# oso95/Agentainer-lab

Measured on AMD Instinct MI355X. Metric: concurrent_agent_chat_req_per_s, higher is better.
Workload: dtype bf16; 1 GPU; model=llama3-8b, agents_per_gpu=64, agents=64, global_batch=64, prompt_len=256, gen_len=57, seq_len=313, parallelism=dp1

## Files before the change

### agentainer_amd/models/llama.py

```python

from __future__ import annotations

import math
from dataclasses import dataclass
from typing import Dict, List, Optional

import torch
import torch.nn.functional as F

from .. import ops


@dataclass
class LlamaConfig:
    name: str = "tiny-llama"
    vocab_size: int = 512
    hidden_size: int = 512
    n_layers: int = 2
    n_heads: int = 4
    n_kv_heads: int = 1
    head_dim: int = 128
    intermediate_size: int = 1024
    rope_theta: float = 500000.0
    max_position: int = 8192
# ... 2 lines not shown
    qkv_bias: bool = False

    @property
    def q_size(self):
        return self.n_heads * self.head_dim

    @property
    def kv_size(self):
        return self.n_kv_heads * self.head_dim

    def kv_bytes_per_token(self, dtype_bytes: int = 2) -> int:
        return 2 * self.n_layers * self.n_kv_heads * self.head_dim * dtype_bytes


@dataclass
class AttnMetadata:

    page_table: torch.Tensor
    seq_lens: torch.Tensor
    slot_mapping: torch.Tensor
    positions: torch.Tensor
    is_prefill: bool = False
    query_starts: Optional[torch.Tensor] = None
    query_lens: Optional[torch.Tensor] = None
    max_qlen: int = 0


class LlamaAttention(torch.nn.Module):
    def __init__(self, cfg: LlamaConfig, tp_rank: int = 0, tp_size: int = 1):
        super().__init__()
        assert cfg.n_heads % tp_size == 0, "n_heads must divide tp_size"
        assert cfg.n_kv_heads % tp_size == 0 or tp_size == 1, \
            "n_kv_heads must divide tp_size"
        self.cfg = cfg
        self.tp_size = tp_size
        self.n_heads = cfg.n_heads // tp_size
        self.n_kv = max(cfg.n_kv_heads // tp_size, 1)
        self.head_dim = cfg.head_dim
        self.scale = 1.0 / math.sqrt(cfg.head_dim)
        q_out = self.n_heads * cfg.head_dim
        kv_out = self.n_kv * cfg.head_dim
        self.qkv_proj = torch.nn.Parameter(
            torch.empty(q_out + 2 * kv_out, cfg.hidden_size, dtype=torch.bfloat16))
        self.o_proj = torch.nn.Parameter(
            torch.empty(cfg.hidden_size, q_out, dtype=torch.bfloat16))
        self.qkv_bias = (torch.nn.Parameter(
            torch.zeros(q_out + 2 * kv_out, dtype=torch.bfloat16))
            if cfg.qkv_bias else None)
        self.qkv_packed = None
        self.o_packed = None
        self.qkv_q = None
        self.o_q = None

    def forward(self, h, k_cache, v_cache, md: AttnMetadata, cos_sin, tp_group=None):
        T = h.size(0)
        if self.qkv_q is not None and T <= 64 and h.is_cuda:
            qkv = ops.linear_quant(h, self.qkv_q)
        else:
            qkv = ops.linear(h, self.qkv_proj, self.qkv_packed)
        if self.qkv_bias is not None:
            qkv = qkv + self.qkv_bias
        q_sz = self.n_heads * self.head_dim
        kv_sz = self.n_kv * self.head_dim
        q = qkv[:, :q_sz].view(T, self.n_heads, self.head_dim)
        k = qkv[:, q_sz:q_sz + kv_sz].view(T, self.n_kv, self.head_dim)
        v = qkv[:, q_sz + kv_sz:].view(T, self.n_kv, self.head_dim)
        ops.rope_append(q, k, v, k_cache, v_cache, cos_sin, md.positions,
                        md.slot_mapping)
        out = torch.empty(T, self.n_heads, self.head_dim, dtype=q.dtype,
                          device=q.device)
        if md.is_prefill:
            ops.paged_prefill_attention(out, q, k_cache, v_cache, md.page_table,
                                        md.seq_lens, md.query_starts,
                                        md.query_lens, self.scale,
                                        max_qlen=md.max_qlen)
        else:
            ops.paged_decode_attention(out, q, k_cache, v_cache, md.page_table,
                                       md.seq_lens, self.scale)
        if self.o_q is not None and T <= 64 and h.is_cuda:
            o = ops.linear_quant(out.view(T, q_sz), self.o_q)
        else:
            o = ops.linear(out.view(T, q_sz), self.o_proj, self.o_packed)
        if tp_group is not None:
            torch.distributed.all_reduce(o, group=tp_group)
        return o


class LlamaMLP(torch.nn.Module):
    def __init__(self, cfg: LlamaConfig, tp_size: int = 1):
        super().__init__()
        inter = cfg.intermediate_size // tp_size
        self.gate_up = torch.nn.Parameter(
            torch.empty(2 * inter, cfg.hidden_size, dtype=torch.bfloat16))
        self.down = torch.nn.Parameter(
            torch.empty(cfg.hidden_size, inter, dtype=torch.bfloat16))
        self.inter = inter
        self.gate_up_packed = None
        self.down_packed = None
        self.gate_up_q = None
        self.down_q = None

    def forward(self, h, tp_group=None):
        turbo = self.gate_up_q is not None and h.size(0) <= 64 and h.is_cuda
        if turbo:
            gu = ops.linear_quant(h, self.gate_up_q)
        else:
            gu = ops.linear(h, self.gate_up, self.gate_up_packed)
        gate, up = gu[:, :self.inter], gu[:, self.inter:]
        act = torch.empty(gu.size(0), self.inter, dtype=gu.dtype,
                          device=gu.device)
        ops.silu_mul(act, gate, up)
        if turbo:
            out = ops.linear_quant(act, self.down_q)
        else:
            out = ops.linear(act, self.down, self.down_packed)
        if tp_group is not None:
            torch.distributed.all_reduce(out, group=tp_group)
        return out


class LlamaLayer(torch.nn.Module):
    def __init__(self, cfg: LlamaConfig, tp_rank: int = 0, tp_size: int = 1):
        super().__init__()
        self.attn = LlamaAttention(cfg, tp_rank, tp_size)
        self.mlp = LlamaMLP(cfg, tp_size)
        self.input_ln = torch.nn.Parameter(torch.empty(cfg.hidden_size, dtype=torch.bfloat16))
        self.post_ln = torch.nn.Parameter(torch.empty(cfg.hidden_size, dtype=torch.bfloat16))
        self.eps = cfg.norm_eps

    def forward(self, hidden, residual, k_cache, v_cache, md, cos_sin, tp_group=None):
        normed = torch.empty_like(hidden)
        if residual is None:
            residual = hidden.clone()
            ops.rmsnorm(normed, hidden, self.input_ln, self.eps)
        else:
            ops.fused_add_rmsnorm(normed, hidden, residual, self.input_ln, self.eps)
        attn_out = self.attn(normed, k_cache, v_cache, md, cos_sin, tp_group)
        normed2 = torch.empty_like(hidden)
        ops.fused_add_rmsnorm(normed2, attn_out, residual, self.post_ln, self.eps)
        mlp_out = self.mlp(normed2, tp_group)
        return mlp_out, residual


class LlamaForCausalLM(torch.nn.Module):
    def __init__(self, cfg: LlamaConfig, device="cpu", tp_rank: int = 0,
                 tp_size: int = 1, seed: int = 0):
        super().__init__()
        self.cfg = cfg
        self.tp_rank = tp_rank
        self.tp_size = tp_size
        self.tp_group = None
        with torch.device(device):
            self.embed = torch.nn.Parameter(
                torch.empty(cfg.vocab_size, cfg.hidden_size, dtype=torch.bfloat16))
            self.layers = torch.nn.ModuleList(
                [LlamaLayer(cfg, tp_rank, tp_size) for _ in range(cfg.n_layers)])
            self.final_ln = torch.nn.Parameter(
                torch.empty(cfg.hidden_size, dtype=torch.bfloat16))
            if cfg.tie_embeddings:
                self.lm_head = self.embed
            else:
                self.lm_head = torch.nn.Parameter(
                    torch.empty(cfg.vocab_size, cfg.hidden_size, dtype=torch.bfloat16))
        self.register_buffer(
            "cos_sin",
            ops.make_cos_sin_table(cfg.max_position, cfg.head_dim, cfg.rope_theta,
                                   device=device),
            persistent=False)
        self.random_init(seed)

    @torch.no_grad()
    def random_init(self, seed: int = 0):
        dev = self.embed.device
        gen = torch.Generator(device=dev).manual_seed(seed)
        for name, p in self.named_parameters():
            if p.dim() >= 2:
                p.data.normal_(0.0, 0.02, generator=gen)
            else:
                p.fill_(1.0)

    @torch.no_grad()
    def forward(self, input_ids: torch.Tensor, md: AttnMetadata,
                kv_caches: List, last_rows: Optional[torch.Tensor] = None
                ) -> torch.Tensor:
        hidden = F.embedding(input_ids, self.embed)
        residual = None
        for i, layer in enumerate(self.layers):
            k_cache, v_cache = kv_caches[i]
            hidden, residual = layer(hidden, residual, k_cache, v_cache, md,
                                     self.cos_sin, self.tp_group)
        final = torch.empty_like(hidden)
        ops.fused_add_rmsnorm(final, hidden, residual, self.final_ln, self.cfg.norm_eps)
        if last_rows is not None:
            final = final[last_rows]
        return ops.linear(final, self.lm_head,
                          getattr(self, 'lm_head_packed', None))

    @torch.no_grad()
    def pack_decode_weights(self, dense_quant: str = ""):
        for layer in self.layers:
            if dense_quant == "mxfp4":
                for mod_, wname, qname in (
                        (layer.attn, "qkv_proj", "qkv_q"),
                        (layer.attn, "o_proj", "o_q"),
                        (layer.mlp, "gate_up", "gate_up_q"),
                        (layer.mlp, "down", "down_q")):
                    w = getattr(mod_, wname).data
                    p, sc = ops.quantize_weight_mxfp4(w)
                    setattr(mod_, qname, ("mxfp4", p, sc, w.size(0)))
            elif dense_quant == "fp8":
                for mod_, wname, qname in (
                        (layer.attn, "qkv_proj", "qkv_q"),
                        (layer.attn, "o_proj", "o_q"),
                        (layer.mlp, "gate_up", "gate_up_q"),
                        (layer.mlp, "down", "down_q")):
                    w = getattr(mod_, wname).data
                    p, sw = ops.quantize_weight_fp8(w)
                    setattr(mod_, qname, ("fp8", p, sw, w.size(0)))
            else:
                layer.attn.qkv_packed = ops.pack_weight(layer.attn.qkv_proj.data)
                layer.attn.o_packed = ops.pack_weight(layer.attn.o_proj.data)
                layer.mlp.gate_up_packed = ops.pack_weight(layer.mlp.gate_up.data)
                layer.mlp.down_packed = ops.pack_weight(layer.mlp.down.data)
        self.lm_head_packed = ops.pack_weight(
            self.lm_head.data if isinstance(self.lm_head, torch.nn.Parameter)
            else self.lm_head)

    @torch.no_grad()
    def load_safetensors(self, path: str):
        from safetensors.torch import load_file
        import glob, os

        files = sorted(glob.glob(os.path.join(path, "*.safetensors")))
        if not files:
            raise FileNotFoundError(f"no safetensors under {path}")
        sd = {}
        for f in files:
            sd.update(load_file(f))
        self._load_hf_state_dict(sd)

    @torch.no_grad()
    def _load_hf_state_dict(self, sd: Dict[str, torch.Tensor]):
        cfg = self.cfg
        r, s = self.tp_rank, self.tp_size
# ... 93 lines not shown
```

### agentainer_amd/models/mixtral.py

```python

from __future__ import annotations

from dataclasses import dataclass
from typing import Dict, List, Optional

import torch
import torch.nn.functional as F

from .. import ops
from .llama import AttnMetadata, LlamaAttention, LlamaConfig


@dataclass
class MixtralConfig(LlamaConfig):
    n_experts: int = 8
    top_k: int = 2


class MixtralMoE(torch.nn.Module):

    def __init__(self, cfg: MixtralConfig, ep_rank: int = 0, ep_size: int = 1):
        super().__init__()
        assert cfg.n_experts % ep_size == 0
        self.cfg = cfg
# ... 153 lines not shown
                             device=h.device)
            le = md[:, 1].long()
            for i in range(self.n_local):
                sel = (le == i).nonzero(as_tuple=True)[0]
                if sel.numel() == 0:
                    continue
                xi = xd[sel]
                gu = ops.linear(xi, self.gate_up[i], None)
                gate, up = gu[:, :self.inter], gu[:, self.inter:]
                act = torch.empty(xi.shape[0], self.inter, dtype=gu.dtype,
                                  device=gu.device)
                ops.silu_mul(act, gate, up)
                eo = ops.linear(act, self.down[i], None)
                yd[sel] = md[sel, 2].unsqueeze(1) * eo.float()
            results.append(yd.to(h.dtype).contiguous())
        returned = self._exchange(results, ep_group)
        out_shard = torch.zeros(ts, H, dtype=torch.float32, device=h.device)
        for d in range(world):
            md = send_meta[d]
            if md.shape[0]:
                out_shard.index_add_(0, md[:, 0].long(),
                                     returned[d].float())
        shards = [None] * world
        sizes = [base + (1 if r < rem else 0) for r in range(world)]
        out_shard = out_shard.to(h.dtype)
        if dist.get_backend(ep_group) == "nccl" and len(set(sizes)) == 1:
            full = torch.empty(T, H, dtype=h.dtype, device=h.device)
            dist.all_gather_into_tensor(full.view(world, -1).view(-1),
                                        out_shard.contiguous(), group=ep_group)
            return full
        dist.all_gather_object(shards, out_shard.cpu(), group=ep_group)
        return torch.cat([s.to(h.device) for s in shards], dim=0)


class MixtralLayer(torch.nn.Module):
    def __init__(self, cfg: MixtralConfig, tp_rank: int = 0, tp_size: int = 1):
        super().__init__()
        self.attn = LlamaAttention(cfg, tp_rank, tp_size)
        self.moe = MixtralMoE(cfg, ep_rank=tp_rank, ep_size=tp_size)
        self.input_ln = torch.nn.Parameter(
            torch.empty(cfg.hidden_size, dtype=torch.bfloat16))
        self.post_ln = torch.nn.Parameter(
            torch.empty(cfg.hidden_size, dtype=torch.bfloat16))
        self.eps = cfg.norm_eps

    def forward(self, hidden, residual, k_cache, v_cache, md, cos_sin,
                tp_group=None):
        normed = torch.empty_like(hidden)
        if residual is None:
            residual = hidden.clone()
            ops.rmsnorm(normed, hidden, self.input_ln, self.eps)
        else:
            ops.fused_add_rmsnorm(normed, hidden, residual, self.input_ln, self.eps)
        attn_out = self.attn(normed, k_cache, v_cache, md, cos_sin, tp_group)
        normed2 = torch.empty_like(hidden)
        ops.fused_add_rmsnorm(normed2, attn_out, residual, self.post_ln, self.eps)
        moe_out = self.moe(normed2, ep_group=tp_group)
        return moe_out, residual


class MixtralForCausalLM(torch.nn.Module):
    def __init__(self, cfg: MixtralConfig, device="cpu", tp_rank: int = 0,
                 tp_size: int = 1, seed: int = 0):
        super().__init__()
        self.cfg = cfg
        self.tp_rank = tp_rank
        self.tp_size = tp_size
        self.tp_group = None
        with torch.device(device):
            self.embed = torch.nn.Parameter(
                torch.empty(cfg.vocab_size, cfg.hidden_size, dtype=torch.bfloat16))
            self.layers = torch.nn.ModuleList(
                [MixtralLayer(cfg, tp_rank, tp_size) for _ in range(cfg.n_layers)])
            self.final_ln = torch.nn.Parameter(
                torch.empty(cfg.hidden_size, dtype=torch.bfloat16))
            self.lm_head = torch.nn.Parameter(
                torch.empty(cfg.vocab_size, cfg.hidden_size, dtype=torch.bfloat16))
        self.register_buffer(
            "cos_sin",
            ops.make_cos_sin_table(cfg.max_position, cfg.head_dim,
                                   cfg.rope_theta, device=device),
            persistent=False)
        self.random_init(seed)

    @torch.no_grad()
    def random_init(self, seed: int = 0):
        dev = self.embed.device
        gen = torch.Generator(device=dev).manual_seed(seed)
        for name, p in self.named_parameters():
            if p.dim() >= 2:
                p.data.normal_(0.0, 0.02, generator=gen)
            else:
                p.fill_(1.0)

    @torch.no_grad()
    def pack_decode_weights(self, expert_fp8: bool = False,
                            expert_fp4: bool = False):
        for layer in self.layers:
            layer.attn.qkv_packed = ops.pack_weight(layer.attn.qkv_proj.data)
            layer.attn.o_packed = ops.pack_weight(layer.attn.o_proj.data)
            for i in range(layer.moe.n_local):
                if expert_fp4:
                    layer.moe.gate_up_fp4[i] = ops.quantize_weight_mxfp4(
                        layer.moe.gate_up[i].data)
                    layer.moe.down_fp4[i] = ops.quantize_weight_mxfp4(
                        layer.moe.down[i].data)
                elif expert_fp8:
# ... 59 lines not shown
```

### agentainer_amd/ops/__init__.py

```python

from __future__ import annotations

import os
from typing import Optional

import torch

from . import reference

_hip = None
_hip_err: Optional[str] = None


def _load_hip():
    global _hip, _hip_err
    if _hip is not None or _hip_err is not None:
        return _hip
    so = os.path.join(os.path.dirname(__file__), "_hip_ops.so")
    if not os.path.exists(so):
        _hip_err = f"HIP extension not built ({so} missing); run python -m agentainer_amd.ops.build"
        return None
    try:
        import importlib.util

        spec = importlib.util.spec_from_file_location("agentainer_amd.ops._hip_ops", so)
        mod = importlib.util.module_from_spec(spec)
        spec.loader.exec_module(mod)
        _hip = mod
    except Exception as exc:
        _hip_err = f"HIP extension failed to load: {exc}"
    return _hip


def hip_available() -> bool:
    return _load_hip() is not None


def _dispatch(name: str, *tensors: torch.Tensor):
    if tensors[0].is_cuda:
        mod = _load_hip()
        if mod is None:
            raise RuntimeError(
                f"op {name!r} on GPU requires the gfx950 HIP extension: {_hip_err}")
        return mod
    return None


def rmsnorm(out, x, w, eps: float = 1e-5):
    mod = _dispatch("rmsnorm", x)
    if mod:
        mod.rmsnorm(out, x, w, float(eps))
    else:
        reference.rmsnorm(out, x, w, eps)
    return out


def fused_add_rmsnorm(out, x, residual, w, eps: float = 1e-5):
    mod = _dispatch("fused_add_rmsnorm", x)
    if mod:
        mod.fused_add_rmsnorm(out, x, residual, w, float(eps))
    else:
        reference.fused_add_rmsnorm(out, x, residual, w, eps)
    return out


def silu_mul(out, gate, up):
    mod = _dispatch("silu_mul", gate)
    if mod:
        mod.silu_mul(out, gate, up)
    else:
        reference.silu_mul(out, gate, up)
    return out


make_cos_sin_table = reference.make_cos_sin_table


def rope_inplace(q, k, cos_sin, positions):
    mod = _dispatch("rope_inplace", q)
    if mod:
        mod.rope_inplace(q, k, cos_sin, positions)
    else:
        reference.rope_inplace(q, k, cos_sin, positions)


def rope_append(q, k, v, k_cache, v_cache, cos_sin, positions, slot_mapping):
    mod = _dispatch("rope_append", q)
    if mod:
        mod.rope_append(q, k, v, k_cache, v_cache, cos_sin, positions,
                        slot_mapping)
    else:
        reference.rope_inplace(q, k, cos_sin, positions)
        reference.kv_append(k_cache, v_cache, k, v, slot_mapping)


def kv_append(k_cache, v_cache, k, v, slot_mapping):
    mod = _dispatch("kv_append", k)
    if mod:
        mod.kv_append(k_cache, v_cache, k, v, slot_mapping)
    else:
        reference.kv_append(k_cache, v_cache, k, v, slot_mapping)


def paged_decode_attention(out, q, k_cache, v_cache, page_table, seq_lens,
                           scale: float):
    mod = _dispatch("paged_decode_attention", q)
    if mod:
        mod.paged_decode_attention(out, q, k_cache, v_cache, page_table,
                                   seq_lens, float(scale))
    else:
        reference.paged_decode_attention(out, q, k_cache, v_cache, page_table,
                                         seq_lens, scale)
    return out


def paged_prefill_attention(out, q, k_cache, v_cache, page_table, seq_lens,
                            query_starts, query_lens, scale: float,
                            max_qlen: int = 0):
    mod = _dispatch("paged_prefill_attention", q)
    if mod:
        mod.paged_prefill_attention(out, q, k_cache, v_cache, page_table,
                                    seq_lens, query_starts, query_lens,
                                    float(scale), int(max_qlen))
    else:
        reference.paged_prefill_attention(out, q, k_cache, v_cache, page_table,
                                          seq_lens, query_starts, query_lens,
                                          scale)
    return out


def greedy_sample(out, logits):
    mod = _dispatch("greedy_sample", logits)
    if mod:
        mod.greedy_sample(out, logits)
    else:
        reference.greedy_sample(out, logits)
    return out


def topp_sample(out, logits, temps, top_ps, seeds):
    mod = _dispatch("topp_sample", logits)
    if mod:
        mod.topp_sample(out, logits, temps, top_ps, seeds)
    else:
        reference.topp_sample(out, logits, temps, top_ps, seeds)
    return out


_ws_cache = {}
_EMPTY_WS = {}
SKINNY_DISABLED = os.environ.get("AGENTAINER_DISABLE_SKINNY", "0") == "1"
SKINNY_FORCED = os.environ.get("AGENTAINER_FORCE_SKINNY", "0") == "1"
_SKINNY_SHAPES = {
    (4096, 4096): (4, 128),
    (4096, 14336): (8, 128),
}
SKINNY_NT = os.environ.get("AGENTAINER_SKINNY_NT", "0") == "1"
SKINNY_KC = int(os.environ.get("AGENTAINER_SKINNY_KC", "0"))
for _spec in os.environ.get("AGENTAINER_SKINNY_SHAPES", "").split(","):
    if _spec.strip():
        _n, _k, _s, _c = (int(v) for v in _spec.split(":"))
        _SKINNY_SHAPES[(_n, _k)] = (_s, _c)


def _skinny_split(ntiles: int, K: int) -> int:
    split = 1
    while split < 16 and ntiles * split < 256 and K % (256 * split * 2) == 0:
        split *= 2
    return split


def pack_weight(w: torch.Tensor) -> torch.Tensor:
    N, K = w.shape
    assert N % 16 == 0 and K % 32 == 0
    p = w.view(N // 16, 16, K // 32, 4, 8).permute(0, 2, 3, 1, 4).contiguous()
    return p.view(-1)


def _skinny_ws(device, N: int, split: int) -> torch.Tensor:
    if split > 1:
        key = (device, N, split)
        ws = _ws_cache.get(key)
        if ws is None or ws.numel() < split * 64 * N:
            ws = torch.empty(split * 64 * N, dtype=torch.float32, device=device)
            _ws_cache[key] = ws
        return ws
    ws = _EMPTY_WS.get(device)
    if ws is None:
        ws = torch.empty(1, dtype=torch.float32, device=device)
        _EMPTY_WS[device] = ws
    return ws


def linear(x: torch.Tensor, w: torch.Tensor,
           w_packed: Optional[torch.Tensor] = None) -> torch.Tensor:
    M, K = x.shape
    N = w.size(0)
    tuned = _SKINNY_SHAPES.get((N, K))
    if (x.is_cuda and M <= 64 and N % 64 == 0 and K % 256 == 0
            and (tuned is not None or SKINNY_FORCED) and not SKINNY_DISABLED):
        mod = _dispatch("skinny_gemm", x)
        split, kc = tuned if tuned else (_skinny_split(N // 64, K), 128)
        if SKINNY_KC:
            kc = SKINNY_KC
        if K % (kc * split):
            split = _skinny_split(N // 64, K)
        out = torch.empty(M, N, dtype=x.dtype, device=x.device)
        ws = _skinny_ws(x.device, N, split)
        if w_packed is not None:
            mod.skinny_gemm_packed(out, x.contiguous(), w_packed, N, K, ws,
                                   split, SKINNY_NT, kc)
        else:
            mod.skinny_gemm(out, x.contiguous(), w, ws, split)
        return out
    return torch.nn.functional.linear(x, w)


def quantize_weight_fp8(w: torch.Tensor):
    N, K = w.shape
    sw = w.float().abs().amax(dim=1).clamp(min=1e-8) / 448.0
    scaled = (w.float() / sw[:, None]).clamp(-448.0, 448.0)
    try:
        w8 = scaled.to(torch.float8_e4m3fn).view(torch.uint8)
    except (RuntimeError, TypeError):
        w8 = scaled.cpu().to(torch.float8_e4m3fn).view(torch.uint8).to(w.device)
    packed = (w8.view(N // 16, 16, K // 32, 4, 8)
              .permute(0, 2, 3, 1, 4).contiguous().view(-1))
    return packed, sw.float().contiguous()


def linear_fp8(x: torch.Tensor, w_packed: torch.Tensor, sw: torch.Tensor,
               N: int) -> torch.Tensor:
    M, K = x.shape
    mod = _dispatch("skinny_gemm_fp8", x)
    assert mod is not None, "linear_fp8 is GPU-only"
    xc = x.contiguous()
    x8 = torch.empty(M, K, dtype=torch.uint8, device=x.device)
    sx = torch.empty(M, dtype=torch.float32, device=x.device)
    mod.quant_fp8_rows(x8, sx, xc)
    split = _skinny_split(N // 64, K)
    ws = _skinny_ws(x.device, N, split)
    out = torch.empty(M, N, dtype=x.dtype, device=x.device)
    mod.skinny_gemm_fp8(out, x8, sx, w_packed, sw, N, K, ws, split)
    return out


_FP4_GRID = torch.tensor([0.0, 0.5, 1.0, 1.5, 2.0, 3.0, 4.0, 6.0])
MXFP4_COMBO = int(os.environ.get("AGENTAINER_MXFP4_COMBO", "0"))


def quantize_weight_mxfp4(w: torch.Tensor):
    N, K = w.shape
    assert N % 16 == 0 and K % 128 == 0, "MXFP4: N%16==0, K%128==0"
    wf = w.float().view(N, K // 32, 32)
    amax = wf.abs().amax(dim=-1).clamp(min=1e-8)
    e = torch.ceil(torch.log2(amax / 6.0)).clamp(-127, 127)
    scale = torch.pow(2.0, e)
    q = wf / scale.unsqueeze(-1)
    mids = torch.tensor([0.25, 0.75, 1.25, 1.75, 2.5, 3.5, 5.0],
                        device=wf.device)
    idx = torch.bucketize(q.abs().contiguous(), mids)
    codes = (idx + torch.where(q < 0, 8, 0)).to(torch.uint8).view(N, K)
    by = (codes[:, 0::2] | (codes[:, 1::2] << 4))
    byv = by.view(N // 16, 16, K // 128, 4, 16)
    packed = byv.permute(0, 2, 3, 1, 4).contiguous().view(-1)
    e8 = (e + 127).clamp(0, 254).to(torch.uint8).view(N, K // 32)
    scv = e8.view(N // 16, 16, K // 128, 4).permute(0, 2, 3, 1).contiguous()
# ... 56 lines not shown
```

### agentainer_amd/ops/csrc/bindings.cpp

```cpp
#include <torch/extension.h>

void rmsnorm(torch::Tensor out, torch::Tensor x, torch::Tensor w, double eps);
void fused_add_rmsnorm(torch::Tensor out, torch::Tensor x,
                       torch::Tensor residual, torch::Tensor w, double eps);
void silu_mul(torch::Tensor out, torch::Tensor gate, torch::Tensor up);
void rope_inplace(torch::Tensor q, torch::Tensor k, torch::Tensor cos_sin,
                  torch::Tensor positions);
void rope_append(torch::Tensor q, torch::Tensor k, torch::Tensor v,
                 torch::Tensor k_cache, torch::Tensor v_cache,
                 torch::Tensor cos_sin, torch::Tensor positions,
                 torch::Tensor slot_mapping);
void kv_append(torch::Tensor k_cache, torch::Tensor v_cache, torch::Tensor k,
               torch::Tensor v, torch::Tensor slot_mapping);
void paged_decode_attention(torch::Tensor out, torch::Tensor q,
                            torch::Tensor k_cache, torch::Tensor v_cache,
                            torch::Tensor page_table, torch::Tensor seq_lens,
                            double scale);
void paged_prefill_attention(torch::Tensor out, torch::Tensor q,
                             torch::Tensor k_cache, torch::Tensor v_cache,
                             torch::Tensor page_table, torch::Tensor seq_lens,
                             torch::Tensor query_starts, torch::Tensor query_lens,
                             double scale, long max_qlen);
void greedy_sample(torch::Tensor out, torch::Tensor logits);
void topp_sample(torch::Tensor out, torch::Tensor logits, torch::Tensor temps,
                 torch::Tensor top_ps, torch::Tensor seeds);
void gather_kv_pages(torch::Tensor dst, torch::Tensor k_cache,
                     torch::Tensor v_cache, torch::Tensor page_ids);
void skinny_gemm(torch::Tensor out, torch::Tensor x, torch::Tensor w,
                 torch::Tensor ws, long split);
void skinny_gemm_packed(torch::Tensor out, torch::Tensor x,
                        torch::Tensor w_packed, long N, long K,
                        torch::Tensor ws, long split, bool nt, long kc);
void quant_fp8_rows(torch::Tensor x8, torch::Tensor sx, torch::Tensor x);
void quant_fp4_rows(torch::Tensor x4, torch::Tensor sx, torch::Tensor x);
void skinny_gemm_mxfp4(torch::Tensor out, torch::Tensor x8, torch::Tensor sx,
                       torch::Tensor w_packed, torch::Tensor w_scales, long N,
                       long K, torch::Tensor ws, long split, long combo);
void skinny_gemm_fp8(torch::Tensor out, torch::Tensor x8, torch::Tensor sx,
                     torch::Tensor w_packed, torch::Tensor sw, long N, long K,
                     torch::Tensor ws, long split);
void mfma_probe(torch::Tensor c, torch::Tensor a, torch::Tensor b);
void scatter_kv_pages(torch::Tensor k_cache, torch::Tensor v_cache,
                      torch::Tensor src, torch::Tensor page_ids);

PYBIND11_MODULE(TORCH_EXTENSION_NAME, m) {
  m.doc() = "agentainer_amd CDNA4 (gfx950) kernels";
  m.def("rmsnorm", &rmsnorm, "RMSNorm (bf16)");
  m.def("fused_add_rmsnorm", &fused_add_rmsnorm, "residual += x; rmsnorm");
  m.def("silu_mul", &silu_mul, "silu(gate) * up");
  m.def("rope_inplace", &rope_inplace, "apply rotary embedding to q,k in place");
  m.def("rope_append", &rope_append, "fused RoPE + paged KV append");
  m.def("kv_append", &kv_append, "scatter new k/v into the paged KV cache");
  m.def("paged_decode_attention", &paged_decode_attention,
        "single-token GQA attention over the paged KV cache");
  m.def("paged_prefill_attention", &paged_prefill_attention,
        "varlen causal MFMA attention over the paged KV cache");
  m.def("greedy_sample", &greedy_sample, "argmax over vocab per row");
  m.def("topp_sample", &topp_sample, "temperature + top-p sampling per row");
  m.def("gather_kv_pages", &gather_kv_pages, "pages -> host-shaped buffer");
  m.def("skinny_gemm", &skinny_gemm, "out[M,N] = x[M,K] @ W[N,K]^T, M<=64");
  m.def("skinny_gemm_packed", &skinny_gemm_packed, "packed-weight skinny GEMM");
  m.def("skinny_gemm_mxfp4", &skinny_gemm_mxfp4, "MXFP4 block-scaled expert GEMM");
  m.def("quant_fp4_rows", &quant_fp4_rows, "per-row e2m1 activation quant");
  m.def("quant_fp8_rows", &quant_fp8_rows, "per-row bf16 -> e4m3 quant");
  m.def("skinny_gemm_fp8", &skinny_gemm_fp8, "fp8 MFMA skinny GEMM");
  m.def("mfma_probe", &mfma_probe, "single 16x16x32 bf16 MFMA on prepacked fragments");
  m.def("scatter_kv_pages", &scatter_kv_pages, "buffer -> pages");
}
```

### agentainer_amd/ops/csrc/rmsnorm.hip

```cpp

#include <torch/extension.h>
#include <ATen/hip/HIPContext.h>
#include "common.h"

namespace {

template <bool FUSED_ADD, int VPT>
__global__ __launch_bounds__(512) void rmsnorm_kernel(
    short* __restrict__ out, const short* __restrict__ x,
    short* __restrict__ residual, const short* __restrict__ w, float eps,
    int H) {
  const int row = blockIdx.x;
  const int tid = threadIdx.x;
  const long base = (long)row * H;
  __shared__ float red[8];

  bf16x8 v[VPT];
  float ss = 0.f;
#pragma unroll
  for (int r = 0; r < VPT; ++r) {
    const int i = (tid + r * 512) * 8;
    if (i < H) {
      v[r] = *reinterpret_cast<const bf16x8*>(x + base + i);
      if (FUSED_ADD) {
        bf16x8 rv = *reinterpret_cast<const bf16x8*>(residual + base + i);
#pragma unroll
        for (int j = 0; j < 8; ++j)
          v[r][j] = f2bits(bits2f(v[r][j]) + bits2f(rv[j]));
        *reinterpret_cast<bf16x8*>(residual + base + i) = v[r];
      }
#pragma unroll
      for (int j = 0; j < 8; ++j) {
        const float f = bits2f(v[r][j]);
        ss = fmaf(f, f, ss);
      }
    } else {
      v[r] = bf16x8{};
    }
  }
  ss = wave_sum(ss);
  if ((tid & (WAVE - 1)) == 0) red[tid / WAVE] = ss;
  __syncthreads();
  ss = 0.f;
#pragma unroll
  for (int wv = 0; wv < 8; ++wv) ss += red[wv];
  const float rms = rsqrtf(ss / (float)H + eps);

#pragma unroll
  for (int r = 0; r < VPT; ++r) {
    const int i = (tid + r * 512) * 8;
    if (i < H) {
      bf16x8 wv = *reinterpret_cast<const bf16x8*>(w + i);
      bf16x8 ov;
#pragma unroll
      for (int j = 0; j < 8; ++j)
        ov[j] = f2bits(bits2f(v[r][j]) * rms * bits2f(wv[j]));
      *reinterpret_cast<bf16x8*>(out + base + i) = ov;
    }
  }
}

}

void rmsnorm(torch::Tensor out, torch::Tensor x, torch::Tensor w, double eps) {
  TORCH_CHECK(x.is_contiguous() && out.is_contiguous() && w.is_contiguous());
  TORCH_CHECK(x.scalar_type() == at::kBFloat16, "rmsnorm: bf16 only");
  const int H = x.size(-1);
  TORCH_CHECK(H % 8 == 0, "hidden size must be a multiple of 8");
  const int T = x.numel() / H;
  auto stream = at::hip::getCurrentHIPStream();
#define RN_LAUNCH(VPT)                                                         \
  hipLaunchKernelGGL((rmsnorm_kernel<false, VPT>), dim3(T), dim3(512), 0,      \
                     stream, (short*)out.data_ptr(),                           \
                     (const short*)x.data_ptr(), nullptr,                      \
                     (const short*)w.data_ptr(), (float)eps, H)
  if (H <= 4096) RN_LAUNCH(1);
  else if (H <= 8192) RN_LAUNCH(2);
  else if (H <= 16384) RN_LAUNCH(4);
  else TORCH_CHECK(false, "rmsnorm: hidden > 16384 unsupported");
#undef RN_LAUNCH
}

void fused_add_rmsnorm(torch::Tensor out, torch::Tensor x,
                       torch::Tensor residual, torch::Tensor w, double eps) {
  TORCH_CHECK(x.is_contiguous() && out.is_contiguous() && w.is_contiguous() &&
              residual.is_contiguous());
  TORCH_CHECK(x.scalar_type() == at::kBFloat16, "fused_add_rmsnorm: bf16 only");
  const int H = x.size(-1);
  TORCH_CHECK(H % 8 == 0, "hidden size must be a multiple of 8");
  const int T = x.numel() / H;
  auto stream = at::hip::getCurrentHIPStream();
#define RNF_LAUNCH(VPT)                                                        \
  hipLaunchKernelGGL((rmsnorm_kernel<true, VPT>), dim3(T), dim3(512), 0,       \
                     stream, (short*)out.data_ptr(),                           \
                     (const short*)x.data_ptr(), (short*)residual.data_ptr(),  \
                     (const short*)w.data_ptr(), (float)eps, H)
  if (H <= 4096) RNF_LAUNCH(1);
  else if (H <= 8192) RNF_LAUNCH(2);
  else if (H <= 16384) RNF_LAUNCH(4);
  else TORCH_CHECK(false, "rmsnorm: hidden > 16384 unsupported");
#undef RNF_LAUNCH
}
```

### agentainer_amd/ops/csrc/skinny_gemm.hip

```cpp

#include <torch/extension.h>
#include <ATen/hip/HIPContext.h>
#include "common.h"

namespace {

typedef __bf16 bf16v8 __attribute__((ext_vector_type(8)));

template <bool SPLIT, bool FULL>
__global__ __launch_bounds__(256) void skinny_gemm_kernel(
    void* __restrict__ out,
    const short* __restrict__ x,
    const short* __restrict__ w,
    int M, int N, int K, int k_per_split) {
  const int n0 = blockIdx.x * 64 + (threadIdx.x / WAVE) * 16;
  const int split = blockIdx.y;
  const int lane = threadIdx.x % WAVE;
  const int l16 = lane % 16;
  const int lg = lane / 16;
  const int k0 = split * k_per_split;
  const int k1 = min(k0 + k_per_split, K);

  f32x4 acc[4];
#pragma unroll
// ... 50 lines not shown
        acc[ms] = __builtin_amdgcn_mfma_f32_16x16x32_bf16(a[ms], bw[i],
                                                          acc[ms], 0, 0, 0);
    }
    if (has_next) stage_write(buf ^ 1);
    __syncthreads();
    buf ^= 1;
  }

#pragma unroll
  for (int ms = 0; ms < 4; ++ms) {
#pragma unroll
    for (int r = 0; r < 4; ++r) {
      const int row = ms * 16 + lg * 4 + r;
      if (row >= M) continue;
      const int col = blockIdx.x * 64 + (threadIdx.x / WAVE) * 16 + l16;
      if (SPLIT) {
        float* o = reinterpret_cast<float*>(out);
        o[((long)split * M + row) * N + col] = acc[ms][r];
      } else {
        short* o = reinterpret_cast<short*>(out);
        o[(long)row * N + col] = f2bits(acc[ms][r]);
      }
    }
  }
}

__global__ __launch_bounds__(256) void splitk_combine_kernel(
    short* __restrict__ out, const float* __restrict__ ws, long mn, int S) {
  const long i4 = ((long)blockIdx.x * blockDim.x + threadIdx.x) * 4;
  if (i4 >= mn) return;
  if (i4 + 4 <= mn) {
    f32x4 acc = *reinterpret_cast<const f32x4*>(ws + i4);
    for (int s = 1; s < S; ++s) {
      const f32x4 v = *reinterpret_cast<const f32x4*>(ws + (long)s * mn + i4);
#pragma unroll
      for (int j = 0; j < 4; ++j) acc[j] += v[j];
    }
    bf16x4 o;
#pragma unroll
    for (int j = 0; j < 4; ++j) o[j] = f2bits(acc[j]);
    *reinterpret_cast<bf16x4*>(out + i4) = o;
  } else {
    for (long i = i4; i < mn; ++i) {
      float acc = 0.f;
      for (int s = 0; s < S; ++s) acc += ws[(long)s * mn + i];
      out[i] = f2bits(acc);
    }
  }
}

}

void skinny_gemm(torch::Tensor out, torch::Tensor x, torch::Tensor w,
                 torch::Tensor ws, long split) {
  TORCH_CHECK(x.is_contiguous() && w.is_contiguous() && out.is_contiguous());
  TORCH_CHECK(x.scalar_type() == at::kBFloat16 && w.scalar_type() == at::kBFloat16);
  const int M = x.size(0), K = x.size(1), N = w.size(0);
  TORCH_CHECK(w.size(1) == K);
  TORCH_CHECK(M <= 64, "skinny_gemm: M <= 64");
  TORCH_CHECK(N % 64 == 0, "skinny_gemm: N % 64 == 0");
  TORCH_CHECK(K % 256 == 0, "skinny_gemm: K % 256 == 0");
  auto stream = at::hip::getCurrentHIPStream();
  const int ntiles = N / 64;
  TORCH_CHECK(split >= 1 && (K % (256 * split)) == 0,
              "invalid split for K (k slices must be 256-aligned)");
  const int kps = K / (int)split;
  const bool full = (M == 64);
#define SG_LAUNCH(SPLIT_, FULL_, OUTP)                                         \
  hipLaunchKernelGGL((skinny_gemm_kernel<SPLIT_, FULL_>),                      \
                     dim3(ntiles, SPLIT_ ? (int)split : 1), dim3(256), 0,      \
                     stream, OUTP, (const short*)x.data_ptr(),                 \
                     (const short*)w.data_ptr(), M, N, K, kps)
  if (split == 1) {
    if (full) SG_LAUNCH(false, true, out.data_ptr());
    else SG_LAUNCH(false, false, out.data_ptr());
  } else {
    TORCH_CHECK(ws.numel() >= (long)split * M * N,
                "skinny_gemm split-K workspace too small");
    TORCH_CHECK(ws.scalar_type() == at::kFloat);
    if (full) SG_LAUNCH(true, true, ws.data_ptr());
    else SG_LAUNCH(true, false, ws.data_ptr());
    const long mn = (long)M * N;
    hipLaunchKernelGGL(splitk_combine_kernel,
                       dim3((mn + 1023) / 1024), dim3(256), 0, stream,
                       (short*)out.data_ptr(), ws.data_ptr<float>(), mn, split);
  }
#undef SG_LAUNCH
}


namespace {

template <bool SPLIT, bool FULL, bool NT, int KC>
__global__ __launch_bounds__(256) void skinny_gemm_packed_kernel(
    void* __restrict__ out, const short* __restrict__ x,
    const short* __restrict__ wp_packed, int M, int N, int K,
    int k_per_split) {
  const int n_tile = blockIdx.x * 4 + threadIdx.x / WAVE;
  const int split = blockIdx.y;
  const int lane = threadIdx.x % WAVE;
  const int l16 = lane % 16;
  const int lg = lane / 16;
  const int k0 = split * k_per_split;
  const int k1 = min(k0 + k_per_split, K);

  f32x4 acc[4];
#pragma unroll
  for (int ms = 0; ms < 4; ++ms) acc[ms] = f32x4{0.f, 0.f, 0.f, 0.f};

  const short* wp = wp_packed + ((long)n_tile * (K / 32) + k0 / 32) * 512 +
                    lane * 8;

  constexpr int FR = KC / 32;
  constexpr int XS = KC + 8;
  __shared__ short x_lds[2][64 * XS];
  const int s_row = threadIdx.x % 64;
  const int s_col0 = (threadIdx.x / 64) * 8;
  const short* s_xp = x + (long)(FULL ? s_row : min(s_row, M - 1)) * K;
  const bool s_alive = FULL || s_row < M;

  bf16x8 st[FR];
  auto stage_load = [&](int k) {
#pragma unroll
    for (int i = 0; i < FR; ++i) {
      st[i] = bf16x8{};
      if (s_alive)
        st[i] = *reinterpret_cast<const bf16x8*>(s_xp + k + s_col0 + 32 * i);
    }
  };
  auto stage_write = [&](int buf) {
#pragma unroll
    for (int i = 0; i < FR; ++i)
      *reinterpret_cast<bf16x8*>(
          &x_lds[buf][s_row * XS + s_col0 + 32 * i]) = st[i];
  };

  bf16v8 bw_cur[FR], bw_nxt[FR];
  auto w_load = [&](bf16v8 (&dst)[FR], long woff) {
// ... 25 lines not shown

  int buf = 0;
  long woff = (long)FR * 512;
  int k = k0;
  while (true) {
    bool has_next = (k + KC < k1);
    if (has_next) {
      stage_load(k + KC);
      w_load(bw_nxt, woff);
      woff += (long)FR * 512;
    }
    compute(bw_cur, buf);
    if (has_next) stage_write(buf ^ 1);
    __syncthreads();
    buf ^= 1;
    k += KC;
    if (!has_next) break;
    has_next = (k + KC < k1);
    if (has_next) {
      stage_load(k + KC);
      w_load(bw_cur, woff);
      woff += (long)FR * 512;
    }
    compute(bw_nxt, buf);
    if (has_next) stage_write(buf ^ 1);
    __syncthreads();
    buf ^= 1;
    k += KC;
    if (!has_next) break;
  }

#pragma unroll
  for (int ms = 0; ms < 4; ++ms) {
#pragma unroll
    for (int r = 0; r < 4; ++r) {
      const int row = ms * 16 + lg * 4 + r;
      if (row >= M) continue;
      const int col = n_tile * 16 + l16;
      if (SPLIT) {
        float* o = reinterpret_cast<float*>(out);
        o[((long)split * M + row) * N + col] = acc[ms][r];
      } else {
        short* o = reinterpret_cast<short*>(out);
        o[(long)row * N + col] = f2bits(acc[ms][r]);
      }
    }
  }
}

}

void skinny_gemm_packed(torch::Tensor out, torch::Tensor x,
                        torch::Tensor w_packed, long N, long K,
                        torch::Tensor ws, long split, bool nt, long kc) {
  TORCH_CHECK(x.is_contiguous() && w_packed.is_contiguous() && out.is_contiguous());
  TORCH_CHECK(x.scalar_type() == at::kBFloat16 &&
              w_packed.scalar_type() == at::kBFloat16);
  const int M = x.size(0);
  TORCH_CHECK(x.size(1) == K);
  TORCH_CHECK(w_packed.numel() == N * K, "packed weight numel mismatch");
  TORCH_CHECK(M <= 64 && N % 64 == 0 && K % 256 == 0);
  TORCH_CHECK(split >= 1 && (K % (256 * split)) == 0);
  auto stream = at::hip::getCurrentHIPStream();
  const int ntiles = (int)N / 64;
  const int kps = (int)K / (int)split;
  const bool full = (M == 64);
  TORCH_CHECK(kc == 128 || kc == 256, "kc must be 128 or 256");
  TORCH_CHECK((K % (kc * split)) == 0, "K must be kc*split aligned");
#define SGP_LAUNCH(SPLIT_, FULL_, NT_, KC_, OUTP)                              \
  hipLaunchKernelGGL((skinny_gemm_packed_kernel<SPLIT_, FULL_, NT_, KC_>),     \
                     dim3(ntiles, SPLIT_ ? (int)split : 1), dim3(256), 0,      \
                     stream, OUTP, (const short*)x.data_ptr(),                 \
                     (const short*)w_packed.data_ptr(), M, (int)N, (int)K, kps)
#define SGP_KC(SPLIT_, FULL_, NT_, OUTP)                                       \
  do {                                                                         \
    if (kc == 128) SGP_LAUNCH(SPLIT_, FULL_, NT_, 128, OUTP);                  \
    else SGP_LAUNCH(SPLIT_, FULL_, NT_, 256, OUTP);                            \
  } while (0)
#define SGP_DISPATCH(SPLIT_, OUTP)                                             \
  do {                                                                         \
    if (full && nt) SGP_KC(SPLIT_, true, true, OUTP);                          \
    else if (full) SGP_KC(SPLIT_, true, false, OUTP);                          \
    else if (nt) SGP_KC(SPLIT_, false, true, OUTP);                            \
    else SGP_KC(SPLIT_, false, false, OUTP);                                   \
  } while (0)
  if (split == 1) {
    SGP_DISPATCH(false, out.data_ptr());
  } else {
    TORCH_CHECK(ws.numel() >= (long)split * M * N && ws.scalar_type() == at::kFloat);
    SGP_DISPATCH(true, ws.data_ptr());
    const long mn = (long)M * N;
    hipLaunchKernelGGL(splitk_combine_kernel, dim3((mn + 1023) / 1024),
                       dim3(256), 0, stream, (short*)out.data_ptr(),
                       ws.data_ptr<float>(), mn, split);
  }
#undef SGP_DISPATCH
#undef SGP_LAUNCH
}


#include <hip/hip_fp8.h>

namespace {

__global__ __launch_bounds__(256) void quant_fp8_rows_kernel(
    unsigned char* __restrict__ x8, float* __restrict__ sx,
    const short* __restrict__ x, int K) {
  const int row = blockIdx.x;
  const short* xp = x + (long)row * K;
  float mx = 0.f;
  for (int i = threadIdx.x * 8; i < K; i += blockDim.x * 8) {
    bf16x8 v = *reinterpret_cast<const bf16x8*>(xp + i);
#pragma unroll
    for (int j = 0; j < 8; ++j) mx = fmaxf(mx, fabsf(bits2f(v[j])));
  }
  mx = wave_max(mx);
  __shared__ float red[4];
  if ((threadIdx.x & 63) == 0) red[threadIdx.x / 64] = mx;
  __syncthreads();
  mx = fmaxf(fmaxf(red[0], red[1]), fmaxf(red[2], red[3]));
  const float scale = fmaxf(mx, 1e-8f) / 448.f;
  const float inv = 1.0f / scale;
  if (threadIdx.x == 0) sx[row] = scale;
  for (int i = threadIdx.x * 8; i < K; i += blockDim.x * 8) {
    bf16x8 v = *reinterpret_cast<const bf16x8*>(xp + i);
    unsigned char o[8];
#pragma unroll
    for (int j = 0; j < 8; ++j) {
      __hip_fp8_e4m3 f8(bits2f(v[j]) * inv);
      o[j] = f8.__x;
    }
    *reinterpret_cast<uint2*>(x8 + (long)row * K + i) =
        *reinterpret_cast<uint2*>(o);
  }
}

template <bool SPLIT>
__global__ __launch_bounds__(256) void skinny_gemm_fp8_kernel(
    void* __restrict__ out,
    const unsigned char* __restrict__ x8,
    const float* __restrict__ sx,
    const unsigned char* __restrict__ wp_packed,
    const float* __restrict__ sw,
    int M, int N, int K, int k_per_split) {
  const int n_tile = blockIdx.x * 4 + threadIdx.x / WAVE;
  const int split = blockIdx.y;
  const int lane = threadIdx.x % WAVE;
// ... 400 lines not shown
```

Measured before the change: 118.5 req/s.

## Fuse split-K partial reduction into the following add+RMSNorm kernel

```diff
diff --git a/agentainer_amd/models/llama.py b/agentainer_amd/models/llama.py
--- a/agentainer_amd/models/llama.py
+++ b/agentainer_amd/models/llama.py
@@ -78,7 +78,8 @@
         self.qkv_q = None
         self.o_q = None
 
-    def forward(self, h, k_cache, v_cache, md: AttnMetadata, cos_sin, tp_group=None):
+    def forward(self, h, k_cache, v_cache, md: AttnMetadata, cos_sin,
+                tp_group=None, defer_reduce: bool = False):
         T = h.size(0)
         if self.qkv_q is not None and T <= 64 and h.is_cuda:
             qkv = ops.linear_quant(h, self.qkv_q)
@@ -105,6 +106,9 @@
                                        md.seq_lens, self.scale)
         if self.o_q is not None and T <= 64 and h.is_cuda:
             o = ops.linear_quant(out.view(T, q_sz), self.o_q)
+        elif defer_reduce and tp_group is None:
+            o = ops.linear_partial(out.view(T, q_sz), self.o_proj,
+                                   self.o_packed)
         else:
             o = ops.linear(out.view(T, q_sz), self.o_proj, self.o_packed)
         if tp_group is not None:
@@ -126,7 +130,7 @@
         self.gate_up_q = None
         self.down_q = None
 
-    def forward(self, h, tp_group=None):
+    def forward(self, h, tp_group=None, defer_reduce: bool = False):
         turbo = self.gate_up_q is not None and h.size(0) <= 64 and h.is_cuda
         if turbo:
             gu = ops.linear_quant(h, self.gate_up_q)
@@ -138,6 +142,8 @@
         ops.silu_mul(act, gate, up)
         if turbo:
             out = ops.linear_quant(act, self.down_q)
+        elif defer_reduce and tp_group is None:
+            out = ops.linear_partial(act, self.down, self.down_packed)
         else:
             out = ops.linear(act, self.down, self.down_packed)
         if tp_group is not None:
@@ -154,17 +160,20 @@
         self.post_ln = torch.nn.Parameter(torch.empty(cfg.hidden_size, dtype=torch.bfloat16))
         self.eps = cfg.norm_eps
 
-    def forward(self, hidden, residual, k_cache, v_cache, md, cos_sin, tp_group=None):
-        normed = torch.empty_like(hidden)
+    def forward(self, hidden, residual, k_cache, v_cache, md, cos_sin,
+                tp_group=None, defer_reduce: bool = False):
         if residual is None:
+            normed = torch.empty_like(hidden)
             residual = hidden.clone()
             ops.rmsnorm(normed, hidden, self.input_ln, self.eps)
         else:
+            normed = torch.empty_like(residual)
             ops.fused_add_rmsnorm(normed, hidden, residual, self.input_ln, self.eps)
-        attn_out = self.attn(normed, k_cache, v_cache, md, cos_sin, tp_group)
-        normed2 = torch.empty_like(hidden)
+        attn_out = self.attn(normed, k_cache, v_cache, md, cos_sin, tp_group,
+                             defer_reduce=True)
+        normed2 = torch.empty_like(residual)
         ops.fused_add_rmsnorm(normed2, attn_out, residual, self.post_ln, self.eps)
-        mlp_out = self.mlp(normed2, tp_group)
+        mlp_out = self.mlp(normed2, tp_group, defer_reduce=defer_reduce)
         return mlp_out, residual
 
 
@@ -214,8 +223,9 @@
         for i, layer in enumerate(self.layers):
             k_cache, v_cache = kv_caches[i]
             hidden, residual = layer(hidden, residual, k_cache, v_cache, md,
-                                     self.cos_sin, self.tp_group)
-        final = torch.empty_like(hidden)
+                                     self.cos_sin, self.tp_group,
+                                     defer_reduce=True)
+        final = torch.empty_like(residual)
         ops.fused_add_rmsnorm(final, hidden, residual, self.final_ln, self.cfg.norm_eps)
         if last_rows is not None:
             final = final[last_rows]
diff --git a/agentainer_amd/models/mixtral.py b/agentainer_amd/models/mixtral.py
--- a/agentainer_amd/models/mixtral.py
+++ b/agentainer_amd/models/mixtral.py
@@ -229,7 +229,8 @@
             ops.rmsnorm(normed, hidden, self.input_ln, self.eps)
         else:
             ops.fused_add_rmsnorm(normed, hidden, residual, self.input_ln, self.eps)
-        attn_out = self.attn(normed, k_cache, v_cache, md, cos_sin, tp_group)
+        attn_out = self.attn(normed, k_cache, v_cache, md, cos_sin, tp_group,
+                             defer_reduce=True)
         normed2 = torch.empty_like(hidden)
         ops.fused_add_rmsnorm(normed2, attn_out, residual, self.post_ln, self.eps)
         moe_out = self.moe(normed2, ep_group=tp_group)
diff --git a/agentainer_amd/ops/__init__.py b/agentainer_amd/ops/__init__.py
--- a/agentainer_amd/ops/__init__.py
+++ b/agentainer_amd/ops/__init__.py
@@ -56,6 +56,11 @@
 
 
 def fused_add_rmsnorm(out, x, residual, w, eps: float = 1e-5):
+    if isinstance(x, SplitKPartial):
+        mod = _dispatch("splitk_add_rmsnorm", residual)
+        mod.splitk_add_rmsnorm(out, x.consume(), x.split, x.M, x.N, residual,
+                               w, float(eps))
+        return out
     mod = _dispatch("fused_add_rmsnorm", x)
     if mod:
         mod.fused_add_rmsnorm(out, x, residual, w, float(eps))
@@ -151,6 +156,8 @@
 _EMPTY_WS = {}
 SKINNY_DISABLED = os.environ.get("AGENTAINER_DISABLE_SKINNY", "0") == "1"
 SKINNY_FORCED = os.environ.get("AGENTAINER_FORCE_SKINNY", "0") == "1"
+SPLITK_DEFER_DISABLED = (
+    os.environ.get("AGENTAINER_DISABLE_SPLITK_DEFER", "0") == "1")
 _SKINNY_SHAPES = {
     (4096, 4096): (4, 128),
     (4096, 14336): (8, 128),
@@ -177,14 +184,44 @@
     return p.view(-1)
 
 
+class _Workspace:
+    __slots__ = ("buf", "gen")
+
+    def __init__(self, buf: torch.Tensor):
+        self.buf = buf
+        self.gen = 0
+
+
+class SplitKPartial:
+    __slots__ = ("ws", "split", "M", "N", "_slot", "_gen")
+
+    def __init__(self, slot: _Workspace, split: int, M: int, N: int):
+        self.ws, self.split, self.M, self.N = slot.buf, split, M, N
+        self._slot, self._gen = slot, slot.gen
+
+    def consume(self) -> torch.Tensor:
+        if self._slot.gen != self._gen or self._slot.buf is not self.ws:
+            raise RuntimeError(
+                "stale SplitKPartial: its split-K workspace was handed out "
+                "again before the partials were consumed")
+        return self.ws
+
+
+def _skinny_ws_slot(device, N: int, split: int) -> _Workspace:
+    stream = torch.cuda.current_stream(device).cuda_stream
+    key = (device, stream, N, split)
+    slot = _ws_cache.get(key)
+    if slot is None or slot.buf.numel() < split * 64 * N:
+        slot = _Workspace(torch.empty(split * 64 * N, dtype=torch.float32,
+                                      device=device))
+        _ws_cache[key] = slot
+    slot.gen += 1
+    return slot
+
+
 def _skinny_ws(device, N: int, split: int) -> torch.Tensor:
     if split > 1:
-        key = (device, N, split)
-        ws = _ws_cache.get(key)
-        if ws is None or ws.numel() < split * 64 * N:
-            ws = torch.empty(split * 64 * N, dtype=torch.float32, device=device)
-            _ws_cache[key] = ws
-        return ws
+        return _skinny_ws_slot(device, N, split).buf
     ws = _EMPTY_WS.get(device)
     if ws is None:
         ws = torch.empty(1, dtype=torch.float32, device=device)
@@ -194,6 +231,15 @@
 
 def linear(x: torch.Tensor, w: torch.Tensor,
            w_packed: Optional[torch.Tensor] = None) -> torch.Tensor:
+    return _linear(x, w, w_packed, False)
+
+
+def linear_partial(x: torch.Tensor, w: torch.Tensor,
+                   w_packed: Optional[torch.Tensor] = None):
+    return _linear(x, w, w_packed, not SPLITK_DEFER_DISABLED)
+
+
+def _linear(x, w, w_packed, defer: bool):
     M, K = x.shape
     N = w.size(0)
     tuned = _SKINNY_SHAPES.get((N, K))
@@ -205,14 +251,20 @@
             kc = SKINNY_KC
         if K % (kc * split):
             split = _skinny_split(N // 64, K)
-        out = torch.empty(M, N, dtype=x.dtype, device=x.device)
-        ws = _skinny_ws(x.device, N, split)
+        defer = defer and split > 1 and M >= 1
+        if defer:
+            slot = _skinny_ws_slot(x.device, N, split)
+            ws = slot.buf
+            out = torch.empty(0, dtype=x.dtype, device=x.device)
+        else:
+            ws = _skinny_ws(x.device, N, split)
+            out = torch.empty(M, N, dtype=x.dtype, device=x.device)
         if w_packed is not None:
             mod.skinny_gemm_packed(out, x.contiguous(), w_packed, N, K, ws,
-                                   split, SKINNY_NT, kc)
+                                   split, SKINNY_NT, kc, not defer)
         else:
-            mod.skinny_gemm(out, x.contiguous(), w, ws, split)
-        return out
+            mod.skinny_gemm(out, x.contiguous(), w, ws, split, not defer)
+        return SplitKPartial(slot, split, M, N) if defer else out
     return torch.nn.functional.linear(x, w)
 
 
diff --git a/agentainer_amd/ops/csrc/bindings.cpp b/agentainer_amd/ops/csrc/bindings.cpp
--- a/agentainer_amd/ops/csrc/bindings.cpp
+++ b/agentainer_amd/ops/csrc/bindings.cpp
@@ -27,10 +27,14 @@
 void gather_kv_pages(torch::Tensor dst, torch::Tensor k_cache,
                      torch::Tensor v_cache, torch::Tensor page_ids);
 void skinny_gemm(torch::Tensor out, torch::Tensor x, torch::Tensor w,
-                 torch::Tensor ws, long split);
+                 torch::Tensor ws, long split, bool combine);
 void skinny_gemm_packed(torch::Tensor out, torch::Tensor x,
                         torch::Tensor w_packed, long N, long K,
-                        torch::Tensor ws, long split, bool nt, long kc);
+                        torch::Tensor ws, long split, bool nt, long kc,
+                        bool combine);
+void splitk_add_rmsnorm(torch::Tensor out, torch::Tensor ws, long split,
+                        long M, long N, torch::Tensor residual,
+                        torch::Tensor w, double eps);
 void quant_fp8_rows(torch::Tensor x8, torch::Tensor sx, torch::Tensor x);
 void quant_fp4_rows(torch::Tensor x4, torch::Tensor sx, torch::Tensor x);
 void skinny_gemm_mxfp4(torch::Tensor out, torch::Tensor x8, torch::Tensor sx,
@@ -58,8 +62,15 @@
   m.def("greedy_sample", &greedy_sample, "argmax over vocab per row");
   m.def("topp_sample", &topp_sample, "temperature + top-p sampling per row");
   m.def("gather_kv_pages", &gather_kv_pages, "pages -> host-shaped buffer");
-  m.def("skinny_gemm", &skinny_gemm, "out[M,N] = x[M,K] @ W[N,K]^T, M<=64");
-  m.def("skinny_gemm_packed", &skinny_gemm_packed, "packed-weight skinny GEMM");
+  m.def("splitk_add_rmsnorm", &splitk_add_rmsnorm,
+        "residual += bf16(sum_s ws[s]); rmsnorm");
+  m.def("skinny_gemm", &skinny_gemm, "out[M,N] = x[M,K] @ W[N,K]^T, M<=64",
+        py::arg("out"), py::arg("x"), py::arg("w"), py::arg("ws"),
+        py::arg("split"), py::arg("combine") = true);
+  m.def("skinny_gemm_packed", &skinny_gemm_packed, "packed-weight skinny GEMM",
+        py::arg("out"), py::arg("x"), py::arg("w_packed"), py::arg("N"),
+        py::arg("K"), py::arg("ws"), py::arg("split"), py::arg("nt"),
+        py::arg("kc"), py::arg("combine") = true);
   m.def("skinny_gemm_mxfp4", &skinny_gemm_mxfp4, "MXFP4 block-scaled expert GEMM");
   m.def("quant_fp4_rows", &quant_fp4_rows, "per-row e2m1 activation quant");
   m.def("quant_fp8_rows", &quant_fp8_rows, "per-row bf16 -> e4m3 quant");
diff --git a/agentainer_amd/ops/csrc/rmsnorm.hip b/agentainer_amd/ops/csrc/rmsnorm.hip
--- a/agentainer_amd/ops/csrc/rmsnorm.hip
+++ b/agentainer_amd/ops/csrc/rmsnorm.hip
@@ -4,6 +4,34 @@
 #include "common.h"
 
 namespace {
+
+template <int VPT>
+__device__ __forceinline__ void rms_scale_store(
+    short* __restrict__ out, const short* __restrict__ w,
+    const bf16x8 (&v)[VPT], float ss, long base, int H, float eps) {
+  __shared__ float red[8];
+  const int tid = threadIdx.x;
+  ss = wave_sum(ss);
+  if ((tid & (WAVE - 1)) == 0) red[tid / WAVE] = ss;
+  __syncthreads();
+  ss = 0.f;
+#pragma unroll
+  for (int wv = 0; wv < 8; ++wv) ss += red[wv];
+  const float rms = rsqrtf(ss / (float)H + eps);
+
+#pragma unroll
+  for (int r = 0; r < VPT; ++r) {
+    const int i = (tid + r * 512) * 8;
+    if (i < H) {
+      bf16x8 wv = *reinterpret_cast<const bf16x8*>(w + i);
+      bf16x8 ov;
+#pragma unroll
+      for (int j = 0; j < 8; ++j)
+        ov[j] = f2bits(bits2f(v[r][j]) * rms * bits2f(wv[j]));
+      *reinterpret_cast<bf16x8*>(out + base + i) = ov;
+    }
+  }
+}
 
 template <bool FUSED_ADD, int VPT>
 __global__ __launch_bounds__(512) void rmsnorm_kernel(
@@ -13,7 +41,6 @@
   const int row = blockIdx.x;
   const int tid = threadIdx.x;
   const long base = (long)row * H;
-  __shared__ float red[8];
 
   bf16x8 v[VPT];
   float ss = 0.f;
@@ -38,26 +65,75 @@
       v[r] = bf16x8{};
     }
   }
-  ss = wave_sum(ss);
-  if ((tid & (WAVE - 1)) == 0) red[tid / WAVE] = ss;
-  __syncthreads();
-  ss = 0.f;
-#pragma unroll
-  for (int wv = 0; wv < 8; ++wv) ss += red[wv];
-  const float rms = rsqrtf(ss / (float)H + eps);
-
+  rms_scale_store<VPT>(out, w, v, ss, base, H, eps);
+}
+
+template <int VPT, int S_CT>
+__global__ __launch_bounds__(512) void splitk_add_rmsnorm_kernel(
+    short* __restrict__ out, const float* __restrict__ ws,
+    short* __restrict__ residual, const short* __restrict__ w, float eps,
+    int H, int S, long slab) {
+  const int row = blockIdx.x;
+  const int tid = threadIdx.x;
+  const long base = (long)row * H;
+
+  bf16x8 v[VPT];
+  float ss = 0.f;
 #pragma unroll
   for (int r = 0; r < VPT; ++r) {
     const int i = (tid + r * 512) * 8;
-    if (i < H) {
-      bf16x8 wv = *reinterpret_cast<const bf16x8*>(w + i);
-      bf16x8 ov;
-#pragma unroll
-      for (int j = 0; j < 8; ++j)
-        ov[j] = f2bits(bits2f(v[r][j]) * rms * bits2f(wv[j]));
-      *reinterpret_cast<bf16x8*>(out + base + i) = ov;
+    const bool alive = i < H;
+    const long off = base + (alive ? i : 0);
+    const float* p = ws + off;
+    f32x4 lo, hi;
+    if constexpr (S_CT > 0) {
+      f32x4 pl[S_CT], ph[S_CT];
+#pragma unroll
+      for (int s = 0; s < S_CT; ++s) {
+        pl[s] = *reinterpret_cast<const f32x4*>(p + s * slab);
+        ph[s] = *reinterpret_cast<const f32x4*>(p + s * slab + 4);
+      }
+      lo = pl[0];
+      hi = ph[0];
+#pragma unroll
+      for (int s = 1; s < S_CT; ++s) {
+#pragma unroll
+        for (int j = 0; j < 4; ++j) {
+          lo[j] += pl[s][j];
+          hi[j] += ph[s][j];
+        }
+      }
+    } else {
+      lo = *reinterpret_cast<const f32x4*>(p);
+      hi = *reinterpret_cast<const f32x4*>(p + 4);
+      for (int s = 1; s < S; ++s) {
+        const f32x4 a = *reinterpret_cast<const f32x4*>(p + s * slab);
+        const f32x4 b = *reinterpret_cast<const f32x4*>(p + s * slab + 4);
+#pragma unroll
+        for (int j = 0; j < 4; ++j) {
+          lo[j] += a[j];
+          hi[j] += b[j];
+        }
+      }
+    }
+    const bf16x8 rv = *reinterpret_cast<const bf16x8*>(residual + off);
+#pragma unroll
+    for (int j = 0; j < 8; ++j) {
+      const short xb = f2bits(j < 4 ? lo[j & 3] : hi[j & 3]);
+      v[r][j] = f2bits(bits2f(xb) + bits2f(rv[j]));
+    }
+    if (alive) {
+      *reinterpret_cast<bf16x8*>(residual + off) = v[r];
+#pragma unroll
+      for (int j = 0; j < 8; ++j) {
+        const float f = bits2f(v[r][j]);
+        ss = fmaf(f, f, ss);
+      }
+    } else {
+      v[r] = bf16x8{};
     }
   }
+  rms_scale_store<VPT>(out, w, v, ss, base, H, eps);
 }
 
 }
@@ -101,3 +177,43 @@
   else TORCH_CHECK(false, "rmsnorm: hidden > 16384 unsupported");
 #undef RNF_LAUNCH
 }
+
+void splitk_add_rmsnorm(torch::Tensor out, torch::Tensor ws, long split,
+                        long M, long N, torch::Tensor residual,
+                        torch::Tensor w, double eps) {
+  TORCH_CHECK(out.is_contiguous() && ws.is_contiguous() &&
+              residual.is_contiguous() && w.is_contiguous());
+  TORCH_CHECK(ws.scalar_type() == at::kFloat,
+              "splitk_add_rmsnorm: f32 partials");
+  TORCH_CHECK(out.scalar_type() == at::kBFloat16 &&
+                  residual.scalar_type() == at::kBFloat16 &&
+                  w.scalar_type() == at::kBFloat16,
+              "splitk_add_rmsnorm: bf16 only");
+  const int H = residual.size(-1);
+  TORCH_CHECK(N == H, "splitk_add_rmsnorm: GEMM N must equal the hidden size");
+  TORCH_CHECK(H % 8 == 0, "hidden size must be a multiple of 8");
+  TORCH_CHECK(M >= 1 && residual.numel() == M * N && out.numel() == M * N &&
+                  w.numel() == H,
+              "splitk_add_rmsnorm: shape mismatch");
+  TORCH_CHECK(split >= 1 && ws.numel() >= split * M * N,
+              "splitk_add_rmsnorm: split-K workspace too small");
+  auto stream = at::hip::getCurrentHIPStream();
+#define SKN_LAUNCH(VPT, S_CT)                                                  \
+  hipLaunchKernelGGL((splitk_add_rmsnorm_kernel<VPT, S_CT>), dim3((int)M),     \
+                     dim3(512), 0, stream, (short*)out.data_ptr(),             \
+                     ws.data_ptr<float>(), (short*)residual.data_ptr(),        \
+                     (const short*)w.data_ptr(), (float)eps, H, (int)split,    \
+                     (long)(M * N))
+#define SKN_SPLIT(VPT)                                                         \
+  do {                                                                         \
+    if (split == 4) SKN_LAUNCH(VPT, 4);                                        \
+    else if (split == 8) SKN_LAUNCH(VPT, 8);                                   \
+    else SKN_LAUNCH(VPT, 0);                                                   \
+  } while (0)
+  if (H <= 4096) SKN_SPLIT(1);
+  else if (H <= 8192) SKN_SPLIT(2);
+  else if (H <= 16384) SKN_SPLIT(4);
+  else TORCH_CHECK(false, "rmsnorm: hidden > 16384 unsupported");
+#undef SKN_SPLIT
+#undef SKN_LAUNCH
+}
diff --git a/agentainer_amd/ops/csrc/skinny_gemm.hip b/agentainer_amd/ops/csrc/skinny_gemm.hip
--- a/agentainer_amd/ops/csrc/skinny_gemm.hip
+++ b/agentainer_amd/ops/csrc/skinny_gemm.hip
@@ -126,7 +126,7 @@
 }
 
 void skinny_gemm(torch::Tensor out, torch::Tensor x, torch::Tensor w,
-                 torch::Tensor ws, long split) {
+                 torch::Tensor ws, long split, bool combine) {
   TORCH_CHECK(x.is_contiguous() && w.is_contiguous() && out.is_contiguous());
   TORCH_CHECK(x.scalar_type() == at::kBFloat16 && w.scalar_type() == at::kBFloat16);
   const int M = x.size(0), K = x.size(1), N = w.size(0);
@@ -146,6 +146,7 @@
                      stream, OUTP, (const short*)x.data_ptr(),                 \
                      (const short*)w.data_ptr(), M, N, K, kps)
   if (split == 1) {
+    TORCH_CHECK(out.numel() >= (long)M * N, "skinny_gemm: out smaller than [M,N]");
     if (full) SG_LAUNCH(false, true, out.data_ptr());
     else SG_LAUNCH(false, false, out.data_ptr());
   } else {
@@ -154,10 +155,14 @@
     TORCH_CHECK(ws.scalar_type() == at::kFloat);
     if (full) SG_LAUNCH(true, true, ws.data_ptr());
     else SG_LAUNCH(true, false, ws.data_ptr());
-    const long mn = (long)M * N;
-    hipLaunchKernelGGL(splitk_combine_kernel,
-                       dim3((mn + 1023) / 1024), dim3(256), 0, stream,
-                       (short*)out.data_ptr(), ws.data_ptr<float>(), mn, split);
+    if (combine) {
+      const long mn = (long)M * N;
+      TORCH_CHECK(out.numel() >= mn, "skinny_gemm: out smaller than [M,N]");
+      hipLaunchKernelGGL(splitk_combine_kernel,
+                         dim3((mn + 1023) / 1024), dim3(256), 0, stream,
+                         (short*)out.data_ptr(), ws.data_ptr<float>(), mn,
+                         split);
+    }
   }
 #undef SG_LAUNCH
 }
@@ -289,7 +294,8 @@
 
 void skinny_gemm_packed(torch::Tensor out, torch::Tensor x,
                         torch::Tensor w_packed, long N, long K,
-                        torch::Tensor ws, long split, bool nt, long kc) {
+                        torch::Tensor ws, long split, bool nt, long kc,
+                        bool combine) {
   TORCH_CHECK(x.is_contiguous() && w_packed.is_contiguous() && out.is_contiguous());
   TORCH_CHECK(x.scalar_type() == at::kBFloat16 &&
               w_packed.scalar_type() == at::kBFloat16);
@@ -322,14 +328,20 @@
     else SGP_KC(SPLIT_, false, false, OUTP);                                   \
   } while (0)
   if (split == 1) {
+    TORCH_CHECK(out.numel() >= (long)M * N,
+                "skinny_gemm_packed: out smaller than [M,N]");
     SGP_DISPATCH(false, out.data_ptr());
   } else {
     TORCH_CHECK(ws.numel() >= (long)split * M * N && ws.scalar_type() == at::kFloat);
     SGP_DISPATCH(true, ws.data_ptr());
-    const long mn = (long)M * N;
-    hipLaunchKernelGGL(splitk_combine_kernel, dim3((mn + 1023) / 1024),
-                       dim3(256), 0, stream, (short*)out.data_ptr(),
-                       ws.data_ptr<float>(), mn, split);
+    if (combine) {
+      const long mn = (long)M * N;
+      TORCH_CHECK(out.numel() >= mn,
+                  "skinny_gemm_packed: out smaller than [M,N]");
+      hipLaunchKernelGGL(splitk_combine_kernel, dim3((mn + 1023) / 1024),
+                         dim3(256), 0, stream, (short*)out.data_ptr(),
+                         ws.data_ptr<float>(), mn, split);
+    }
   }
 #undef SGP_DISPATCH
 #undef SGP_LAUNCH
```

Result: faster. 120.0 req/s, median of 6 (+1.2%).
